# Rodrigops27/MPC-EKF4FastCharge

Hardware: AMD Instinct MI355X
Metric: MPC+EKF control steps/sec (whole batch), Np=5 Nc=2; 1/2/4/8 MI355X (higher is better)
Workload: dtype f64

## Files before the change

### mpc-ekf4fastcharge_amd/csrc/mpcekf_host.cpp

```cpp
#include <hip/hip_runtime.h>

#include <sched.h>

#include <algorithm>
#include <cmath>
#include <condition_variable>
#include <cstdarg>
#include <cstdio>
#include <cstdlib>
#include <cstring>
#include <deque>
#include <mutex>
#include <new>
#include <string>
#include <thread>
#include <vector>

#include "../../include/mpcekf.h"
#include "mpcekf_eig.hpp"
#include "mpcekf_kernels.hpp"
#include "mpcekf_summary.hpp"
#include "mpcekf_thermal.hpp"

using namespace mk;
// ... 142 lines not shown
  int NM = 0, nz = 0, nzp = 0;
  int ncon = 0, ncon_dev = 0, sw = 7;
  bool initialized = false;
  KRom r{};
  KCfg k{};
  KState s{};
  mpcekf_config cfg{};
  double *d_cell_blob = nullptr, *d_plant_blob = nullptr, *d_bulk = nullptr, *d_poly = nullptr;
  double *d_const = nullptr;
  double *d_mb = nullptr;
  bool mb = false;
  double *d_scal = nullptr;
  int *d_int = nullptr;
  double *d_prob = nullptr;
  double *d_zk = nullptr, *d_zbk = nullptr;
  double *d_bnd = nullptr;
  int *d_xm = nullptr;
  double *d_xg = nullptr;
  bool split_cell = false;
  bool quad = false;
  int ekf4_block = 256;
  int *d_ts = nullptr;
  double *d_hist = nullptr;
  long long *d_stamps = nullptr;
  bool wide = false;
  KWide w{};
  double *d_lin = nullptr, *d_zsoc = nullptr;
  std::vector<double> h_lim;
  double *d_lim = nullptr;
  bool percell = false;
  const double *lim() const { return percell ? d_lim : nullptr; }
  double *d_sum = nullptr, *d_sum_reach = nullptr, *d_sum_obs = nullptr;
  char *d_sum_ring = nullptr;
  int32_t sum_slot = -1;
  size_t sum_row() const { return (((size_t)SUM_WIN * (size_t)n * 8) + 255) & ~(size_t)255; }
  double *d_th = nullptr, *d_th_par = nullptr, *d_th_i = nullptr, *d_th_ocv = nullptr;
  int32_t th_nocv = 0;
  double *d_uk1p = nullptr;
  int flush_period = LAZY_H;
  bool flush_roll = false;
  hipStream_t fstream = nullptr;
  hipEvent_t ev_fork = nullptr, ev_join = nullptr;
  bool bounds_side = false;
  hipEvent_t ev_bfork = nullptr, ev_bjoin = nullptr;
  double *d_tmp = nullptr;
  size_t tmp_bytes = 0;
// ... 700 lines not shown
      (rc = dalloc(&X->d_zk, n * (X->nz + 2))) || (rc = dalloc(&X->d_zbk, n * (X->nz + 2))) ||
      (rc = dalloc(&X->d_bnd, n * NBND)) || (rc = dalloc(&X->d_xg, n * 4)) ||
      (rc = hipMalloc((void **)&X->d_xm, n * 4 * sizeof(int)) == hipSuccess ? 0 : MPCEKF_E_HIP) ||
      (rc = dalloc(&X->d_ts, n * NM * 2)) || (rc = dalloc(&X->d_hist, n * LAZY_H * 2)) ||
      (X->mb && (rc = dalloc(&X->d_mb, n * MBREC)))
#ifdef MPCEKF_STAMPS
      || (rc = dalloc(&X->d_stamps, n * NSTAMPS))
#endif
  ) {
    mpcekf_ctx_destroy(X);
    return rc;
  }
  double *sc = X->d_scal;
  s.SOCn = sc; s.SOCp = sc + n; s.x0 = sc + 2 * n; s.S0 = sc + 3 * n; s.priorI = sc + 4 * n;
  s.uk_1 = sc + 5 * n; s.uk = sc + 6 * n; s.vk = sc + 7 * n; s.J_unc = sc + 8 * n; s.J_fin = sc + 9 * n;
  s.warn = X->d_int; s.status = X->d_int + n; s.nviol = X->d_int + 2 * n; s.hflag = X->d_int + 3 * n;
  s.hslow = X->d_int + 4 * n;
  HIPCHK(hipMemset(s.hslow, 0, sizeof(int)));
  s.prob = X->d_prob;
  s.ts_ekf = X->d_ts; s.ts_plant = X->d_ts + n * NM;
  s.hist_p = X->d_hist; s.hist_u = X->d_hist + n * LAZY_H;
  s.mb = X->d_mb;
  s.stamps = X->d_stamps;
  if (X->d_stamps) HIPCHK(hipMemset(X->d_stamps, 0, (size_t)n * NSTAMPS * sizeof(long long)));
  double *cs = X->d_const;
  s.Tc = cs; s.SOC0 = cs + n; s.SOC0n = cs + 2 * n; s.SOC0p = cs + 3 * n;
  if (X->sw != 7 && ((rc = dalloc(&X->d_lin, n * MPCEKF_LIN_SIZE)) || (rc = dalloc(&X->d_zsoc, n)))) {
    mpcekf_ctx_destroy(X);
    return rc;
  }
  if (X->wide) {
    KWide &w = X->w;
    w.Np = cfg->Np; w.Nc = cfg->Nc; w.ncon = X->ncon;
    const size_t nc = (size_t)X->ncon;
    if ((rc = dalloc(&w.prob, n * wide_prob_doubles(w.Np, w.Nc))) || (rc = dalloc(&w.X, nc * n * w.Nc)) ||
        (rc = dalloc(&w.R, (size_t)n * (w.Nc * (w.Nc + 1) / 2))) || (rc = dalloc(&w.K, nc * n)) || (rc = dalloc(&w.hii, nc * n)) || (rc = dalloc(&w.it, n)) ||
        (rc = dalloc(&w.smin, (size_t)w.Nc * w.Nc + 1)) || (rc = dalloc(&X->d_lin, n * MPCEKF_LIN_SIZE)) ||
        (rc = dalloc(&w.q, 1)) || (rc = dalloc(&w.list, n)) || (rc = dalloc(&w.hist, 128)) ||
        (rc = dalloc(&X->d_zsoc, n))) {
      mpcekf_ctx_destroy(X);
      return rc;
    }
    HIPCHK(hipMemset(w.q, 0, sizeof(int)));
    HIPCHK(hipMemset(w.hist, 0, 128 * sizeof(int)));
    HIPCHK(hipMemset(w.it, 0, n * sizeof(int)));
    rc = launch_wide_smin(w, -rom->Ts / (3600 * rom->Q), rom->A, X->stream);
// ... 2 lines not shown
  }
  *out = X;
  return MPCEKF_OK;
}

int mpcekf_ctx_destroy(mpcekf_ctx *X) {
  if (!X) return MPCEKF_OK;
  (void)hipSetDevice(X->device);
  if (X->stream) (void)X->drain();
  if (X->fstream) (void)hipStreamSynchronize(X->fstream);
  delete X->copier;
  X->copier = nullptr;
  for (hipEvent_t e : X->xev) (void)hipEventDestroy(e);
  for (hipEvent_t e : X->ev) (void)hipEventDestroy(e);
  if (X->ev_fork) (void)hipEventDestroy(X->ev_fork);
  if (X->ev_join) (void)hipEventDestroy(X->ev_join);
  if (X->ev_bfork) (void)hipEventDestroy(X->ev_bfork);
  if (X->ev_bjoin) (void)hipEventDestroy(X->ev_bjoin);
  void *ptrs[] = {X->d_prob, X->d_cell_blob, X->d_plant_blob, X->d_bulk, X->d_const, X->d_scal, X->d_int, X->d_zk,
                  X->d_zbk,       X->d_tmp,        X->s.bigx, X->s.ekf,   X->s.lam,   X->d_ts, X->d_hist, X->d_stamps, X->d_bnd, X->d_xm, X->d_xg,
                  X->w.prob, X->w.X, X->w.R, X->w.K, X->w.hii, X->w.it, X->w.smin, X->d_lin, X->d_zsoc, X->d_mb, X->d_uk1p,
                  X->w.q, X->w.list, X->w.hist, X->d_poly, X->d_szk, X->d_sxg, X->d_sxm, X->d_slin, X->d_sv, X->d_zslot,
                  X->d_obs_blob, X->d_obs, X->d_obs_plan, X->d_lim, X->d_sum, X->d_sum_reach, X->d_sum_obs,
                  X->d_sum_ring, X->d_th, X->d_th_par, X->d_th_i, X->d_th_ocv};
  for (void *p : ptrs)
    if (p) (void)hipFree(p);
  for (auto &g : X->graphs) (void)hipGraphExecDestroy(g.exec);
  if (X->h_bounce) (void)hipHostFree(X->h_bounce);
  if (X->fstream) (void)hipStreamDestroy(X->fstream);
  if (X->stream) (void)hipStreamDestroy(X->stream);
  delete X;
  return MPCEKF_OK;
}

int mpcekf_ctx_config(const mpcekf_ctx *X, mpcekf_config *cfg) {
  if (!X || !cfg) return fail(MPCEKF_E_ARG, "ctx_config: null argument");
  *cfg = X->cfg;
  return MPCEKF_OK;
}

int mpcekf_ctx_info(const mpcekf_ctx *X, int64_t *ncells, int32_t *nmodels, int32_t *nz, int32_t *ncon) {
  if (!X) return fail(MPCEKF_E_ARG, "null ctx");
  if (ncells) *ncells = X->n;
  if (nmodels) *nmodels = X->NM;
  if (nz) *nz = X->nz;
  if (ncon) *ncon = X->ncon;
  return MPCEKF_OK;
// ... 26 lines not shown
  if (!X || ((!soc0_pct || !tc_degC) && X->n)) return fail(MPCEKF_E_ARG, "init_cells: null argument");
  HIPCHK(hipSetDevice(X->device));
  const size_t n = (size_t)X->n;
  int rc0 = 0;
  if ((X->n && (rc0 = check_tc(tc_degC, n)))) return rc0;
  std::vector<double> cst(n * 8), sc(n * 10, 0.0);
  for (size_t c = 0; c < n; ++c) {
    double tc = tc_degC[c], soc0 = soc0_pct[c];
    double T = tc + 273.15;
    double z = soc0 / 100;
    cst[0 * n + c] = tc;
    cst[1 * n + c] = z;
    cst[2 * n + c] = host_soc(X, 0, z, T);
    cst[3 * n + c] = host_soc(X, 1, z, T);
    sc[0 * n + c] = cst[2 * n + c];
    sc[1 * n + c] = cst[3 * n + c];
    sc[3 * n + c] = X->cfg.SigmaX0[5];
  }
  HIPCHK(hipMemcpyAsync(X->d_const, cst.data(), cst.size() * 8, hipMemcpyHostToDevice, X->stream));
  HIPCHK(hipMemcpyAsync(X->d_scal, sc.data(), sc.size() * 8, hipMemcpyHostToDevice, X->stream));
  HIPCHK(hipMemsetAsync(X->s.lam, 0, n * X->ncon_dev * 8, X->stream));
  HIPCHK(hipMemsetAsync(X->d_int, 0, n * 4 * sizeof(int), X->stream));
  HIPCHK(hipMemsetAsync(X->d_ts, 0, n * X->NM * 2 * sizeof(int), X->stream));
  int rc = launch_init_state(X->n, X->NM, X->s.ekf, X->s.bigx, X->cfg.SigmaX0, X->stream);
  if (rc) return fail(MPCEKF_E_HIP, "init kernel: %s", hipGetErrorString((hipError_t)rc));
  if (X->mb) {
    std::vector<double> mbs(n * MBREC, 0.0);
    for (size_t c = 0; c < n; ++c)
      for (int p = 0; p <= NX; ++p) mbs[c * MBREC + 6 + p * (NX + 1) + p] = X->cfg.SigmaX0[p];
    HIPCHK(hipMemcpyAsync(X->d_mb, mbs.data(), mbs.size() * 8, hipMemcpyHostToDevice, X->stream));
    HIPCHK(hipStreamSynchronize(X->stream));
  }
  HIPCHK(hipStreamSynchronize(X->stream));
  X->initialized = true;
  return MPCEKF_OK;
}

static int need_init(mpcekf_ctx *X) {
  if (!X) return fail(MPCEKF_E_ARG, "null ctx");
  if (!X->initialized) return fail(MPCEKF_E_STATE, "call mpcekf_init_cells first");
  HIPCHK(hipSetDevice(X->device));
  return MPCEKF_OK;
}

static int lerr(int rc, const char *what) {
  if (rc) return fail(MPCEKF_E_HIP, "%s launch: %s", what, hipGetErrorString((hipError_t)rc));
// ... 274 lines not shown
        q.uk = X->s.uk;
        q.iapp = X->d_th_i;
        q.par = X->d_th_par;
        q.ocv = X->d_th_ocv;
        q.rec = X->d_th;
        q.temp = (double *)row(15, k);
        q.heat = (double *)row(16, k);
        q.n = X->n;
        q.nocv = X->th_nocv;
        q.th0n = X->r.th0n;
        q.th100n = X->r.th100n;
        q.Ts = X->r.Ts;
        if ((rc = lerr(launch_thermal(q, X->stream), "thermal"))) return rc;
      }
    }
    return MPCEKF_OK;
  };
  if (capturing) {
    std::vector<uintptr_t> key = {(uintptr_t)nsteps, (uintptr_t)dtc, (uintptr_t)diag, (uintptr_t)bounds};
    for (const F &e : f) key.push_back((uintptr_t)e.dev);
    key.push_back((uintptr_t)osel.plan);
    key.push_back((uintptr_t)nslots);
    key.push_back((uintptr_t)lim);
    for (int i = 0; i < nslots; ++i) key.push_back((uintptr_t)slots[i]);
    key.push_back((uintptr_t)X->d_th_ocv);
    key.push_back((uintptr_t)X->th_nocv);
    key.push_back((uintptr_t)X->d_th);
    key.push_back((uintptr_t)(sum ? X->d_sum_reach : nullptr));
    key.push_back((uintptr_t)(sum ? X->d_sum : nullptr));
    if ((rc = X->graph_launch(key, run_steps))) return rc;
  } else if ((rc = run_steps())) {
    return rc;
  }
  if (!outputs_on_device)
    for (int i = 0; i < NF; ++i)
      if (f[i].host)
        HIPCHK(hipMemcpyAsync(f[i].host, f[i].dev, per * f[i].width * f[i].esz, hipMemcpyDeviceToHost, X->stream));
  if (nsteps > 0 && f[6].dev)
    HIPCHK(hipMemcpyAsync(X->d_zk, row(6, nsteps - 1), n * nzz * 8, hipMemcpyDeviceToDevice, X->stream));
  if (nsteps > 0 && f[7].dev)
    HIPCHK(hipMemcpyAsync(X->d_zbk, row(7, nsteps - 1), n * nzz * 8, hipMemcpyDeviceToDevice, X->stream));
  HIPCHK(hipStreamSynchronize(X->stream));
  if (X->timing) {
    static const int slot[5] = {MPCEKF_K_PLANT, MPCEKF_K_CELL, MPCEKF_K_BOUNDS, MPCEKF_K_HILD, MPCEKF_K_FLUSH};
    static const int e0[5] = {0, 1, 2, 3, 5};
    for (int k = 0; k < nsteps; ++k)
// ... 992 lines not shown
    HIPCHK(xf.out(scal, dc, n * (size_t)nslots * 8));
  }
  if (warn) HIPCHK(xf.out(warn, X->s.warn, n * 4));
  if (status) HIPCHK(xf.out(status, X->s.status, n * 4));
  return xf.end(async);
}
int mpcekf_get_scalars(mpcekf_ctx *X, const int32_t *slots, int32_t nslots, double *scal, int32_t *warn,
                       int32_t *status) {
  return get_scalars_impl(X, slots, nslots, scal, warn, status, false);
}
int mpcekf_get_scalars_async(mpcekf_ctx *X, const int32_t *slots, int32_t nslots, double *scal, int32_t *warn,
                             int32_t *status) {
  return get_scalars_impl(X, slots, nslots, scal, warn, status, true);
}

int mpcekf_set_state(mpcekf_ctx *X, const mpcekf_state *st) {
  if (X) X->stage_zk = X->stage_lin = X->stage_v = X->stage_obs = false;
  int rc = need_init(X);
  if (rc) return rc;
  if (!st) return fail(MPCEKF_E_ARG, "set_state: null");
  const size_t n = (size_t)X->n, NM = (size_t)X->NM, nc = (size_t)X->ncon, ncd = (size_t)X->ncon_dev;
  if (st->bigX) HIPCHK(hipMemcpyAsync(X->s.bigx, st->bigX, n * NM * 6 * 8, hipMemcpyHostToDevice, X->stream));
  if (st->ekf) HIPCHK(hipMemcpyAsync(X->s.ekf, st->ekf, n * NM * REC * 8, hipMemcpyHostToDevice, X->stream));
  if (st->mb && X->mb) HIPCHK(hipMemcpyAsync(X->d_mb, st->mb, n * MBREC * 8, hipMemcpyHostToDevice, X->stream));
  std::vector<double> sc(st->scal ? n * 8 : 0), lam(st->lambda ? n * ncd : 0);
  std::vector<int> iv(st->warn || st->status ? n * 2 : 0);
  if (!iv.empty() && !(st->warn && st->status)) {
    HIPCHK(hipMemcpyAsync(iv.data(), X->d_int, n * 2 * 4, hipMemcpyDeviceToHost, X->stream));
    HIPCHK(hipStreamSynchronize(X->stream));
  }
  for (size_t c = 0; c < n; ++c) {
    if (st->scal)
      for (int k = 0; k < MPCEKF_NSCAL; ++k) sc[kScalMap[k] * n + c] = st->scal[c * MPCEKF_NSCAL + k];
    if (st->lambda)
      for (size_t i = 0, ci = 0; i < ncd; ++i)
        if (row_enabled(X->cfg.Np, X->cfg.Nc, X->sw, (int)i)) lam[i * n + c] = st->lambda[c * nc + ci++];
    if (st->warn) iv[c] = st->warn[c];
    if (st->status) iv[n + c] = st->status[c];
  }
  if (st->scal) HIPCHK(hipMemcpyAsync(X->d_scal, sc.data(), n * 8 * 8, hipMemcpyHostToDevice, X->stream));
  if (st->lambda) HIPCHK(hipMemcpyAsync(X->s.lam, lam.data(), n * ncd * 8, hipMemcpyHostToDevice, X->stream));
  if (!iv.empty()) HIPCHK(hipMemcpyAsync(X->d_int, iv.data(), n * 2 * 4, hipMemcpyHostToDevice, X->stream));
  HIPCHK(hipStreamSynchronize(X->stream));
  return MPCEKF_OK;
}

// ... 2 lines not shown
```

### mpc-ekf4fastcharge_amd/csrc/mpcekf_kernels.hip

```cpp
#include <hip/hip_runtime.h>

#include <cmath>
#include <cstdlib>
#include <cstdint>
#include <type_traits>

#include "mpcekf_kernels.hpp"
#include "mpcekf_mpc.hpp"
#include "mpcekf_hild.hpp"

#pragma clang fp contract(off)

namespace mk {


#ifdef MPCEKF_STAMPS
#define STAMP(i)                                                                          \
  do {                                                                                    \
    if (io.stamps) io.stamps[(size_t)(i) * s.n + c] = (long long)__builtin_amdgcn_s_memtime(); \
  } while (0)
#define STAMPP(i)                                                                                  \
  do {                                                                                             \
    if (s.stamps) s.stamps[(size_t)(12 + (i)) * s.n + c] = (long long)__builtin_amdgcn_s_memtime(); \
  } while (0)
// ... 273 lines not shown
    two_nearest(Zp, nZ, SOC, a, b);
    iZu = a; iZl = b;
    if (Zp[iZu] < Zp[iZl]) { iZu = b; iZl = a; }
  }
  if (nT > 1) {
    int a, b;
    two_nearest(Tp, nT, Tk, a, b);
    iTu = a; iTl = b;
    if (Tp[iTu] < Tp[iTl]) { iTu = b; iTl = a; }
  }
  double aZ = 0.0, aT = 0.0;
  if (nZ > 1) aZ = (SOC - Zp[iZl]) / (Zp[iZu] - Zp[iZl]);
  if (nT > 1) aT = (Tk - Tp[iTl]) / (Tp[iTu] - Tp[iTl]);
  xi.g[0] = (1 - aT) * (1 - aZ);
  xi.g[1] = (1 - aT) * aZ;
  xi.g[2] = aT * (1 - aZ);
  xi.g[3] = aT * aZ;
  xi.m[0] = iTl * nZ + iZl;
  xi.m[1] = iTl * nZ + iZu;
  xi.m[2] = iTu * nZ + iZl;
  xi.m[3] = iTu * nZ + iZu;
}

__device__ __forceinline__ void load_x(const double *rec, double x[NX]) {
  const double2 *p = reinterpret_cast<const double2 *>(rec);
  double2 a = p[0], b = p[1];
  x[0] = a.x; x[1] = a.y; x[2] = b.x; x[3] = b.y;
  x[4] = rec[4];
}
__device__ __forceinline__ void load_rec(const double *rec, double x[NX], double S[NPK]) {
  const double2 *p = reinterpret_cast<const double2 *>(rec);
  double v[REC];
#pragma unroll
  for (int i = 0; i < REC / 2; ++i) {
    double2 t = p[i];
    v[2 * i] = t.x;
    v[2 * i + 1] = t.y;
  }
#pragma unroll
  for (int i = 0; i < NX; ++i) x[i] = v[i];
#pragma unroll
  for (int i = 0; i < NPK; ++i) S[i] = v[NX + i];
}
__device__ __forceinline__ void store_rec(double *rec, const double x[NX], const double S[NPK]) {
  double2 *p = reinterpret_cast<double2 *>(rec);
  double v[REC];
#pragma unroll
  for (int i = 0; i < NX; ++i) v[i] = x[i];
#pragma unroll
  for (int i = 0; i < NPK; ++i) v[NX + i] = S[i];
#pragma unroll
  for (int i = 0; i < REC / 2; ++i) p[i] = make_double2(v[2 * i], v[2 * i + 1]);
}
__device__ __forceinline__ void load_S(const double *rec, double S[NPK]) {
  S[0] = rec[NX];
  const double2 *p = reinterpret_cast<const double2 *>(rec + NX + 1);
#pragma unroll
  for (int i = 0; i < 7; ++i) {
    double2 t = p[i];
    S[1 + 2 * i] = t.x;
    S[2 + 2 * i] = t.y;
  }
}

__device__ __forceinline__ void jacobi5(double a[NPK], double V[NX * NX]) {
#pragma unroll
  for (int i = 0; i < NX * NX; ++i) V[i] = (i % (NX + 1)) == 0 ? 1.0 : 0.0;
  for (int sweep = 0; sweep < 50; ++sweep) {
    double off = 0.0, dg = 0.0;
#pragma unroll
    for (int p = 0; p < NX; ++p) {
      dg = dg + a[pk(p, p)] * a[pk(p, p)];
#pragma unroll
      for (int q = p + 1; q < NX; ++q) off = off + a[pk(p, q)] * a[pk(p, q)];
    }
    if (!(off > 1e-36 * dg)) break;
#pragma unroll
    for (int p = 0; p < NX - 1; ++p) {
#pragma unroll
      for (int q = p + 1; q < NX; ++q) {
        double apq = a[pk(p, q)];
        if (apq != 0.0) {
          double theta = (a[pk(q, q)] - a[pk(p, p)]) / (2.0 * apq);
          double t;
          if (fabs(theta) > 1e150) {
// ... 994 lines not shown
  const int lo = __builtin_amdgcn_readlane((int)b, l), hi = __builtin_amdgcn_readlane((int)(b >> 32), l);
  return __longlong_as_double(((long long)hi << 32) | (long long)(unsigned)lo);
}
__global__ void __launch_bounds__(256) k_flush(const KRom r, const KCfg cf, const KState s, const int t,
                                               const int new_ts, const int64_t c_lo, const int64_t c_hi) {
  const int NM = r.NM;
  const int lane = threadIdx.x & 63;
  const int64_t nw = (int64_t)gridDim.x * (blockDim.x >> 6);
  const int64_t w0 = ((int64_t)blockIdx.x * blockDim.x + threadIdx.x) >> 6;
  const double W = cf.SigmaW;
  const double *cC = r.bulk_tab, *cP = r.bulk_tab + (size_t)NM * REC;
  for (int m0 = 0; m0 < NM; m0 += 64) {
    const int m = m0 + lane;
    const bool act = m < NM;
    const int mm = act ? m : NM - 1;
    double ce[REC], cp[6];
#pragma unroll
    for (int e = 0; e < REC; ++e) ce[e] = cC[(size_t)mm * REC + e];
#pragma unroll
    for (int e = 0; e < 6; ++e) cp[e] = cP[(size_t)mm * 6 + e];
    struct FCell {
      double hpl, hul, xe[REC], xp[6];
      int tse, tsp;
    };
    auto fload = [&](int64_t c, FCell &F) {
      F.hpl = s.hist_p[(size_t)(lane & (LAZY_H - 1)) * s.n + c];
      F.hul = s.hist_u[(size_t)(lane & (LAZY_H - 1)) * s.n + c];
      F.tse = (act && !(cf.flags & KF_MB)) ? s.ts_ekf[c * NM + m] : t;
      F.tsp = act ? s.ts_plant[c * NM + m] : t;
      const double2 *re = reinterpret_cast<const double2 *>(s.ekf + ((size_t)c * NM + mm) * REC);
      const double2 *rp = reinterpret_cast<const double2 *>(s.bigx + ((size_t)c * NM + mm) * 6);
#pragma unroll
      for (int e = 0; e < REC / 2; ++e) {
        const double2 v = re[e];
        F.xe[2 * e] = v.x;
        F.xe[2 * e + 1] = v.y;
      }
#pragma unroll
      for (int e = 0; e < 3; ++e) {
        const double2 v = rp[e];
        F.xp[2 * e] = v.x;
        F.xp[2 * e + 1] = v.y;
      }
    };
    FCell cur;
    if (c_lo + w0 < c_hi) fload(c_lo + w0, cur);
    for (int64_t c = c_lo + w0; c < c_hi; c += nw) {
      FCell nx;
      if (c + nw < c_hi) fload(c + nw, nx);
      const double hpl = cur.hpl, hul = cur.hul;
      const int tse = cur.tse, tsp = cur.tsp;
      double2 *re = reinterpret_cast<double2 *>(s.ekf + ((size_t)c * NM + mm) * REC);
      double2 *rp = reinterpret_cast<double2 *>(s.bigx + ((size_t)c * NM + mm) * 6);
      double *xe = cur.xe, *xp = cur.xp;
      int kmin = min(tse, tsp);
#pragma unroll
      for (int o = 1; o < 64; o <<= 1) kmin = min(kmin, __shfl_xor(kmin, o));
      for (int k = kmin + 1; k <= t; ++k) {
        const int sl = k & (LAZY_H - 1);
        const double p = rl64(hpl, sl), u = rl64(hul, sl);
        if (k > tse) {
#pragma unroll
          for (int e = 0; e < NX; ++e) xe[e] = __builtin_fma(ce[e], xe[e], p);
#pragma unroll
          for (int e = NX; e < REC; ++e) xe[e] = __builtin_fma(ce[e], xe[e], W);
        }
        if (k > tsp) {
#pragma unroll
          for (int e = 0; e < 6; ++e) xp[e] = __builtin_fma(cp[e], xp[e], u);
        }
      }
      if (tse < t) {
#pragma unroll
        for (int e = 0; e < REC / 2; ++e) re[e] = make_double2(xe[2 * e], xe[2 * e + 1]);
      }
      if (tsp < t) {
#pragma unroll
        for (int e = 0; e < 3; ++e) rp[e] = make_double2(xp[2 * e], xp[2 * e + 1]);
      }
      if (act) {
        s.ts_ekf[c * NM + m] = new_ts;
        s.ts_plant[c * NM + m] = new_ts;
      }
      cur = nx;
    }
  }
}

__device__ __forceinline__ void replay_x(double x[NX], const double *a, int ts, int t, double pt, const KState &s,
                                        int64_t c) {
  if (ts + 1 < t) {
    for (int k0 = ts + 1; k0 < t; k0 += RCH) {
      double p[RCH];
      ring_chunk(s.hist_p, s, c, k0, t - 1, p);
#pragma unroll
      for (int i = 0; i < RCH; ++i)
        if (k0 + i < t)
#pragma unroll
          for (int e = 0; e < NX; ++e) x[e] = __builtin_fma(a[e], x[e], p[i]);
    }
  }
  if (ts < t)
#pragma unroll
    for (int e = 0; e < NX; ++e) x[e] = __builtin_fma(a[e], x[e], pt);
}
__device__ __forceinline__ void replay_S(double S[NPK], const double *a, int ts, int t, double W) {
  for (int k = ts + 1; k <= t; ++k) {
#pragma unroll
    for (int i = 0, pp = 0; pp < NX; ++pp)
#pragma unroll
      for (int q = pp; q < NX; ++q, ++i) S[i] = __builtin_fma(a[NX + i], S[i], W);
  }
}

template <int NZ>
__device__ __forceinline__ void ekf_catch_up4(const KState &s, const CellCtx &cc, int NM, const int m[4], int64_t c,
                                              int t, double W, double pt) {
  int ts[4];
#pragma unroll
  for (int j = 0; j < 4; ++j) ts[j] = s.ts_ekf[c * NM + m[j]];
  bool need[4];
#pragma unroll
  for (int j = 0; j < 4; ++j) {
    need[j] = ts[j] < t;
#pragma unroll
    for (int i = 0; i < j; ++i) need[j] = need[j] && m[i] != m[j];
  }
  if (!(need[0] || need[1] || need[2] || need[3])) return;
  double x[4][NX], S[4][NPK];
#pragma unroll
  for (int j = 0; j < 4; ++j)
    if (need[j]) load_rec(cc.erec + (size_t)m[j] * REC, x[j], S[j]);
#pragma unroll
  for (int j = 0; j < 4; ++j) {
    if (!need[j]) continue;
    const double *a = cc.L + m[j] * cc.stride + NZ * NX + NZ;
    for (int k0 = ts[j] + 1; k0 <= t; k0 += RCH) {
      double p[RCH];
      if (k0 < t) ring_chunk(s.hist_p, s, c, k0, t - 1, p);
#pragma unroll
      for (int i = 0; i < RCH; ++i) {
        const int k = k0 + i;
        if (k > t) break;
// ... 471 lines not shown
    }
    if (io.bnd) io.bnd[BD_M * s.n + c] = -1.0;
    if (io.xm_out) {
#pragma unroll
      for (int j = 0; j < 4; ++j) { io.xm_out[c * 4 + j] = xi.m[j]; io.xg_out[c * 4 + j] = xi.g[j]; }
    }
    } else {
    double x0 = s.x0[c] + s.priorI[c];
    double S0 = s.S0[c] + cf.SigmaW;
    const double SOC0 = s.SOC0[c];
    double SOC = SOC0 - x0 * (r.Ts / (3600 * r.Q));
    STAMP(1);
    get_xind(r.nT, r.nZ, Tp, Zp, cc.T, SOC, xi);
    STAMP(2);
    const int t = io.lazy_t;
    bool dup[4];
    int tsj[4];
    double xr[4][NX], Sr[4][NPK];
#pragma unroll
    for (int j = 0; j < 4; ++j) {
      dup[j] = false;
#pragma unroll
      for (int i = 0; i < j; ++i) dup[j] = dup[j] || xi.m[i] == xi.m[j];
      if (j == 0) load_rec(cc.erec + (size_t)xi.m[j] * REC, xr[j], Sr[j]);
      else load_x(cc.erec + (size_t)xi.m[j] * REC, xr[j]);
      tsj[j] = t ? s.ts_ekf[c * r.NM + xi.m[j]] : 0;
    }
    const double pt = t ? (fplant ? s.priorI[c] : s.hist_p[(size_t)(t % LAZY_H) * s.n + c]) : 0.0;
    run_plant();
    if (planted) vk = vplant;
    if (t) {
#pragma unroll
      for (int j = 0; j < 4; ++j)
        if (!dup[j]) replay_x(xr[j], cc.L + xi.m[j] * cc.stride + NZ * NX + NZ, tsj[j], t, pt, s, c);
#pragma unroll
      for (int j = 1; j < 4; ++j)
#pragma unroll
        for (int i = j - 1; i >= 0; --i)
          if (xi.m[i] == xi.m[j])
#pragma unroll
            for (int k = 0; k < NX; ++k) xr[j][k] = xr[i][k];
    }
    STAMP(3);
    KR kr1;
    vhat = get_vars<NZ>(r, cc, xi, ik, x0, SOC0, warn, st, Z, Zsoc, xr, 0, &kr1);
    STAMP(4);
    if (st & ST_ERROR) {
      s.status[c] = st;
      s.warn[c] = warn;
// ... 18 lines not shown
        row[cI] = acc;
      }
      double acc = 0.0;
#pragma unroll
      for (int cI = 0; cI < NX; ++cI) acc = __builtin_fma(row[cI], ChatV[j][cI], acc);
      St[j] = acc + cf.SigmaV;
#pragma unroll
      for (int k = 0; k < NX; ++k) Lg[j][k] = row[k] / St[j];
    }
    double St0 = C0 * S0 * C0 + cf.SigmaV;
    double L0 = S0 * C0 / St0;
    double res = vk - vhat;
#pragma unroll
    for (int j = 0; j < 4; ++j) {
      launder(St[j]);
#pragma unroll
      for (int k = 0; k < NX; ++k) launder(Lg[j][k]);
    }
    __builtin_amdgcn_sched_barrier(0);
    STAMP(5);
    double xu[4][NX];
    double Sn[NPK];
    auto s_ahead = [&](int j) { return j >= 1 && j < 4 && !dup[j]; };
    if (s_ahead(1)) load_S(cc.erec + (size_t)xi.m[1] * REC, Sn);
#pragma unroll
    for (int j = 0; j < 4; ++j) {
      double *rec = cc.erec + (size_t)xi.m[j] * REC;
      double xj[NX], Sj[NPK];
      if (dup[j]) {
        load_rec(rec, xj, Sj);
      } else {
#pragma unroll
        for (int k = 0; k < NX; ++k) xj[k] = xr[j][k];
        if (j == 0) {
#pragma unroll
          for (int k = 0; k < NPK; ++k) Sj[k] = Sr[j][k];
        } else {
#pragma unroll
          for (int k = 0; k < NPK; ++k) Sj[k] = Sn[k];
        }
        if (t && j > 0) replay_S(Sj, cc.L + xi.m[j] * cc.stride + NZ * NX + NZ, tsj[j], t, cf.SigmaW);
      }
      meas_update_regs<false>(xj, Sj, Lg[j], St[j], res);
      if (j + 1 < 4 && s_ahead(j + 1)) load_S(cc.erec + (size_t)xi.m[j + 1] * REC, Sn);
      store_rec(rec, xj, Sj);
      if (t) s.ts_ekf[c * r.NM + xi.m[j]] = t;
#pragma unroll
      for (int k = 0; k < NX; ++k) xu[j][k] = xj[k];
      __builtin_amdgcn_sched_barrier(0);
    }
    STAMP(6);
    x0 = __builtin_fma(L0, res, x0);
    S0 = S0 - L0 * St0 * L0;
    SOC = SOC0 - x0 * (r.Ts / (3600 * r.Q));
    int m1[4];
#pragma unroll
    for (int j = 0; j < 4; ++j) m1[j] = xi.m[j];
    get_xind(r.nT, r.nZ, Tp, Zp, cc.T, SOC, xi);
    const bool same = m1[0] == xi.m[0] && m1[1] == xi.m[1] && m1[2] == xi.m[2] && m1[3] == xi.m[3] &&
                      !(dup[1] || dup[2] || dup[3]);
    if (!same) {
      if (io.lazy_t) ekf_catch_up4<NZ>(s, cc, r.NM, xi.m, c, io.lazy_t, cf.SigmaW, pt);
#pragma unroll
      for (int j = 0; j < 4; ++j) load_x(cc.erec + (size_t)xi.m[j] * REC, xu[j]);
    }
    STAMP(7);
    vhat = get_vars<NZ>(r, cc, xi, ik, x0, SOC0, warn, st, Z, Zsoc, xu, 0, &kr2);
    have_kr2 = true;
    const int jm = corner_max(xi);
#pragma unroll
    for (int k = 0; k < NX; ++k) xmax[k] = jm == 0 ? xu[0][k] : jm == 1 ? xu[1][k] : jm == 2 ? xu[2][k] : xu[3][k];
    have_xmax = true;
    __builtin_amdgcn_sched_barrier(0);
    STAMP(8);
    s.warn[c] = warn;
    if (st & ST_ERROR) {
      s.status[c] = st;
      s.x0[c] = x0;
      s.S0[c] = S0;
      if (fused) s.uk[c] = NaN;
      fail_outputs();
      return;
    }
    if (io.bnd) {
      double *bd = io.bnd;
      const int64_t n = s.n;
#pragma unroll
// ... 24 lines not shown
    }
    }
  }
  if (!(PARTS & (P_MPC | P_LIN))) return;
  if (!(PARTS & P_EKF) && fused) {
    if (st & ST_ERROR) return;
    vk = s.vk[c];
  }

  Lin L;
  if (io.mode & (MODE_LIN | MODE_FUSED)) {
    double zr[NROLE];
    if (fused && (PARTS & P_EKF)) {
#pragma unroll
      for (int q = 0; q < NROLE; ++q) zr[q] = Z[q];
    } else {
      if (!fused && (st & ST_ERROR)) { fail_outputs(); return; }
#pragma unroll
      for (int q = 0; q < NROLE; ++q) zr[q] = io.zk_in[c * (nz + 2) + r.perm[q]];
      Zsoc = io.zk_in[c * (nz + 2) + nz + 1];
#pragma unroll
      for (int j = 0; j < 4; ++j) { xi.m[j] = io.xm_in[c * 4 + j]; xi.g[j] = io.xg_in[c * 4 + j]; }
    }
    mats_handler<NZ>(r, cc, xi, zr, Zsoc, Tc + 273.15, L, MB ? s.x0[c] : 0.0, xmax, fused && (PARTS & P_EKF) && have_xmax,
                     fused && (PARTS & P_EKF) && have_kr2 ? &kr2 : nullptr);
    if (io.lin_out) lin_store(io.lin_out + c * 35, L);
    if (io.x_out)
#pragma unroll
      for (int q = 0; q < 6; ++q) io.x_out[c * 6 + q] = L.xhat[q];
  }
  STAMP(10);
  if (PARTS & P_LIN) {
    if (fused) {
      double acc = 0.0;
#pragma unroll
      for (int k = 0; k < 6; ++k) acc = acc + L.Cphi[k] * L.xhat[k];
      if (io.phise) io.phise[c] = acc + s.uk[c] * L.Dphi + L.bphi;
      if (io.v) io.v[c] = vk;
      if (io.soc) io.soc[c] = Zsoc;
      if (io.zsoc_out) io.zsoc_out[c] = Zsoc;
    }
    return;
  }

  if (io.mode & (MODE_MPC | MODE_FUSED)) {
    if (!fused) {
      if (st & ST_ERROR) { fail_outputs(); return; }
// ... 309 lines not shown
  return (((0.0 + qbc<0>(v)) + qbc<1>(v)) + qbc<2>(v)) + qbc<3>(v);
}

constexpr int BOUNDS_BLOCK = 1024;
__host__ __device__ inline int bounds_c0_base(const KRom &r) { return r.rom_global ? 0 : r.cell_tab + 1; }
template <int NZ, bool GR>
__global__ void __launch_bounds__(BOUNDS_BLOCK) k_bounds(const KRom r, const KState s, const double *bd, double *zbk) {
  extern __shared__ double lds[];
  if (!GR) stage_lds(lds, r.cell_blob, r.cell_tab);
  __syncthreads();
  const double *L = GR ? r.cell_blob : lds;
  const int64_t gt = (int64_t)blockIdx.x * blockDim.x + threadIdx.x;
  const int64_t n = s.n;
  const int j = (int)(gt & 3);
  const int64_t cq = gt >> 2;
  const int64_t c = cq < n ? cq : n - 1;
  const int nz = r.nz;
  const bool valid = cq < n && bd[BD_M * n + c] >= 0.0;
  const double g = bd[(BD_G + j) * n + c];
  const int m = valid ? (int)bd[(BD_M + j) * n + c] : 0;
  const double *Cm = L + m * r.cell_stride;
  const double S0 = bd[BD_S0 * n + c];
  double S1b[NPK];
  load_S(s.ekf + ((size_t)c * r.NM + (valid ? (int)bd[BD_M * n + c] : 0)) * REC, S1b);
#pragma unroll
  for (int k = 0; k < NX; ++k)
#pragma unroll
    for (int l = k + 1; l < NX; ++l) S1b[pk(k, l)] = 2 * S1b[pk(k, l)];
  ChatK K;
  K.Rfn = bd[(BD_K + 0) * n + c];
  K.Rfp = bd[(BD_K + 1) * n + c];
  K.Rctn = bd[(BD_K + 2) * n + c];
  K.Rctp = bd[(BD_K + 3) * n + c];
  K.dUn0 = bd[(BD_K + 4) * n + c];
  K.dUp3 = bd[(BD_K + 5) * n + c];
  double ChV[NX];
  chat_row(r, K, Cm, g, ChV);
  const double ChV0 = bd[BD_C0 * n + c];
  const double res0n = bd[BD_R0N * n + c], res0p = bd[BD_R0P * n + c];
  const double dUn = bd[BD_DUN * n + c], dUp = bd[BD_DUP * n + c];
  const bool ph0pp = rowf(r, R_PHISE0, G_PPHIS);
  double cph0[NX];
#pragma unroll
  for (int k = 0; k < NX; ++k) {
    double v = g * Cm[R_PHISE0 * NX + k];
    if (ph0pp) v = v + ChV[k];
    cph0[k] = v;
// ... 703 lines not shown
```

### mpc-ekf4fastcharge_amd/csrc/mpcekf_kernels.hpp

```cpp
#pragma once
#include <cstddef>
#include <cstdint>

namespace mk {

constexpr int NX = 5;
constexpr int NPK = 15;
constexpr int NA = 7;
constexpr int REC = 20;
constexpr int MAXT = 8;
constexpr int MAXZ = 40;
constexpr int MAXROWS = 64;
constexpr int NPLANT = 9;
constexpr int PREC = NPLANT * NX + NPLANT + NPLANT + 6;
#ifndef MPCEKF_LAZY_H
#define MPCEKF_LAZY_H 64
#endif
constexpr int LAZY_H = MPCEKF_LAZY_H;
constexpr int MAXTT = 8;
constexpr int MBREC = 42;
constexpr int KF_MB = 1 << 8;

enum { R_IFDL0 = 0, R_IFDL3, R_IF0, R_IF3, R_TH0, R_TH3, R_TE1, R_TEE, R_PHIE, R_PHISE0, R_NPHISE2, NROLE };
enum : unsigned { G_NTH = 1, G_PTH = 2, G_NPHISE = 4, G_PPHISE = 8, G_PHIE = 16, G_PHIE0 = 32, G_THETAE = 64,
// ... 29 lines not shown
  int max_warn, max_hild, flags;
};

enum { LK_REF = 0, LK_U_MAX, LK_U_MIN, LK_DU_MIN, LK_DU_MAX, LK_V_MAX, LK_PHISE_MIN, LK_ZMAX, NLIMK };

struct KState {
  int64_t n;
  double *bigx;
  double *ekf;
  double *SOCn, *SOCp, *x0, *S0, *priorI, *uk_1, *uk, *vk;
  double *lam;
  int *warn, *status;
  double *Tc;
  const double *SOC0, *SOC0n, *SOC0p;
  double *J_unc, *J_fin;
  int *nviol;
  int *hflag;
  int *hslow;
  double *prob;
  double *mb;
  int *ts_ekf, *ts_plant;
  double *hist_p, *hist_u;
  long long *stamps;
};

constexpr int OBS_ROW = 8;
constexpr int OBS_MAXROWS = 32;
enum { OBS_PLAIN = 0, OBS_NTHSS, OBS_PTHSS, OBS_NPHISE, OBS_PPHISE, OBS_PHIE, OBS_THETAE, OBS_PPHIS };
enum { OBS_S_NEGSOC = 0, OBS_S_POSSOC, OBS_S_CELLSOC };
struct KObs {
  const double *blob;
  int stride, tab, tablen, len;
  int global;
  int nobs, slot_phie0;
  unsigned desc[OBS_MAXROWS];
  double *rec;
};

enum { OBS_SRC_NEGSOC = -1, OBS_SRC_POSSOC = -2, OBS_SRC_CELLSOC = -3, OBS_SRC_PHIE0 = -4, OBS_SRC_VCELL = -5 };
enum { OBS_NEED_V = 1,
       OBS_NEED_UN = 2,
       OBS_NEED_UP = 4 };
struct KObsSel {
  const int *plan;
  int nsel, need;
  double *out;
};
// ... 98 lines not shown
```

Measured before the change: 252.0 million.

## Cache four active EKF corner records in a coalesced hot buffer

Adds a per-cell hot buffer holding the four currently active interpolation-corner EKF records in a struct-of-arrays layout (stride n), plus their model indices and timestamps. The cell kernel reads and writes these hot slots when the corner set is unchanged, and writes them back to the main per-model record array when the corners change. The lazy flush, xmax lookup and bounds kernels are updated to consult the hot slots. The aim is coalesced global memory access instead of scattered record loads, at the cost of extra index checks, write-back traffic on corner changes, and more complexity around state consistency.

```diff
diff --git a/mpc-ekf4fastcharge_amd/csrc/mpcekf_host.cpp b/mpc-ekf4fastcharge_amd/csrc/mpcekf_host.cpp
--- a/mpc-ekf4fastcharge_amd/csrc/mpcekf_host.cpp
+++ b/mpc-ekf4fastcharge_amd/csrc/mpcekf_host.cpp
@@ -188,6 +188,12 @@
   int ekf4_block = 256;
   int *d_ts = nullptr;
   double *d_hist = nullptr;
+  double *d_hot = nullptr;
+  int *d_hot_i = nullptr;
+  int hot_clear() {
+    if (d_hot_i) HIPCHK(hipMemsetAsync(d_hot_i, 0xFF, (size_t)n * 4 * sizeof(int), stream));
+    return MPCEKF_OK;
+  }
   long long *d_stamps = nullptr;
   bool wide = false;
   KWide w{};
@@ -934,6 +940,25 @@
   s.hist_p = X->d_hist; s.hist_u = X->d_hist + n * LAZY_H;
   s.mb = X->d_mb;
   s.stamps = X->d_stamps;
+  {
+    bool hot = true;
+    if (const char *e = std::getenv("MPCEKF_HOT_CORNERS")) hot = std::atoi(e) != 0;
+    if (hot && !X->mb && !X->quad && !X->flush_roll && n > 0) {
+      if (hipMalloc((void **)&X->d_hot, n * 4 * REC * sizeof(double)) != hipSuccess ||
+          hipMalloc((void **)&X->d_hot_i, n * 8 * sizeof(int)) != hipSuccess) {
+        (void)hipGetLastError();
+        if (X->d_hot) (void)hipFree(X->d_hot);
+        if (X->d_hot_i) (void)hipFree(X->d_hot_i);
+        X->d_hot = nullptr;
+        X->d_hot_i = nullptr;
+      } else {
+        s.hot_rec = X->d_hot;
+        s.hot_m = X->d_hot_i;
+        s.hot_ts = X->d_hot_i + n * 4;
+        if ((rc = X->hot_clear())) { mpcekf_ctx_destroy(X); return rc; }
+      }
+    }
+  }
   if (X->d_stamps) HIPCHK(hipMemset(X->d_stamps, 0, (size_t)n * NSTAMPS * sizeof(long long)));
   double *cs = X->d_const;
   s.Tc = cs; s.SOC0 = cs + n; s.SOC0n = cs + 2 * n; s.SOC0p = cs + 3 * n;
@@ -982,7 +1007,7 @@
                   X->w.prob, X->w.X, X->w.R, X->w.K, X->w.hii, X->w.it, X->w.smin, X->d_lin, X->d_zsoc, X->d_mb, X->d_uk1p,
                   X->w.q, X->w.list, X->w.hist, X->d_poly, X->d_szk, X->d_sxg, X->d_sxm, X->d_slin, X->d_sv, X->d_zslot,
                   X->d_obs_blob, X->d_obs, X->d_obs_plan, X->d_lim, X->d_sum, X->d_sum_reach, X->d_sum_obs,
-                  X->d_sum_ring, X->d_th, X->d_th_par, X->d_th_i, X->d_th_ocv};
+                  X->d_sum_ring, X->d_th, X->d_th_par, X->d_th_i, X->d_th_ocv, X->d_hot, X->d_hot_i};
   for (void *p : ptrs)
     if (p) (void)hipFree(p);
   for (auto &g : X->graphs) (void)hipGraphExecDestroy(g.exec);
@@ -1055,6 +1080,7 @@
   HIPCHK(hipMemsetAsync(X->s.lam, 0, n * X->ncon_dev * 8, X->stream));
   HIPCHK(hipMemsetAsync(X->d_int, 0, n * 4 * sizeof(int), X->stream));
   HIPCHK(hipMemsetAsync(X->d_ts, 0, n * X->NM * 2 * sizeof(int), X->stream));
+  if ((rc0 = X->hot_clear())) return rc0;
   int rc = launch_init_state(X->n, X->NM, X->s.ekf, X->s.bigx, X->cfg.SigmaX0, X->stream);
   if (rc) return fail(MPCEKF_E_HIP, "init kernel: %s", hipGetErrorString((hipError_t)rc));
   if (X->mb) {
@@ -1375,6 +1401,7 @@
     key.push_back((uintptr_t)osel.plan);
     key.push_back((uintptr_t)nslots);
     key.push_back((uintptr_t)lim);
+    key.push_back((uintptr_t)X->s.hot_rec);
     for (int i = 0; i < nslots; ++i) key.push_back((uintptr_t)slots[i]);
     key.push_back((uintptr_t)X->d_th_ocv);
     key.push_back((uintptr_t)X->th_nocv);
@@ -2413,6 +2440,7 @@
   const size_t n = (size_t)X->n, NM = (size_t)X->NM, nc = (size_t)X->ncon, ncd = (size_t)X->ncon_dev;
   if (st->bigX) HIPCHK(hipMemcpyAsync(X->s.bigx, st->bigX, n * NM * 6 * 8, hipMemcpyHostToDevice, X->stream));
   if (st->ekf) HIPCHK(hipMemcpyAsync(X->s.ekf, st->ekf, n * NM * REC * 8, hipMemcpyHostToDevice, X->stream));
+  if ((rc = X->hot_clear())) return rc;
   if (st->mb && X->mb) HIPCHK(hipMemcpyAsync(X->d_mb, st->mb, n * MBREC * 8, hipMemcpyHostToDevice, X->stream));
   std::vector<double> sc(st->scal ? n * 8 : 0), lam(st->lambda ? n * ncd : 0);
   std::vector<int> iv(st->warn || st->status ? n * 2 : 0);
diff --git a/mpc-ekf4fastcharge_amd/csrc/mpcekf_kernels.hip b/mpc-ekf4fastcharge_amd/csrc/mpcekf_kernels.hip
--- a/mpc-ekf4fastcharge_amd/csrc/mpcekf_kernels.hip
+++ b/mpc-ekf4fastcharge_amd/csrc/mpcekf_kernels.hip
@@ -319,18 +319,18 @@
   xi.m[3] = iTu * nZ + iZu;
 }
 
-__device__ __forceinline__ void load_x(const double *rec, double x[NX]) {
+__device__ __forceinline__ void load_x(const double *rec, double x[NX], size_t st = 1) {
   const double2 *p = reinterpret_cast<const double2 *>(rec);
-  double2 a = p[0], b = p[1];
+  double2 a = p[0], b = p[st];
   x[0] = a.x; x[1] = a.y; x[2] = b.x; x[3] = b.y;
-  x[4] = rec[4];
-}
-__device__ __forceinline__ void load_rec(const double *rec, double x[NX], double S[NPK]) {
+  x[4] = reinterpret_cast<const double *>(p + 2 * st)[0];
+}
+__device__ __forceinline__ void load_rec(const double *rec, double x[NX], double S[NPK], size_t st = 1) {
   const double2 *p = reinterpret_cast<const double2 *>(rec);
   double v[REC];
 #pragma unroll
   for (int i = 0; i < REC / 2; ++i) {
-    double2 t = p[i];
+    double2 t = p[i * st];
     v[2 * i] = t.x;
     v[2 * i + 1] = t.y;
   }
@@ -339,7 +339,7 @@
 #pragma unroll
   for (int i = 0; i < NPK; ++i) S[i] = v[NX + i];
 }
-__device__ __forceinline__ void store_rec(double *rec, const double x[NX], const double S[NPK]) {
+__device__ __forceinline__ void store_rec(double *rec, const double x[NX], const double S[NPK], size_t st = 1) {
   double2 *p = reinterpret_cast<double2 *>(rec);
   double v[REC];
 #pragma unroll
@@ -347,17 +347,20 @@
 #pragma unroll
   for (int i = 0; i < NPK; ++i) v[NX + i] = S[i];
 #pragma unroll
-  for (int i = 0; i < REC / 2; ++i) p[i] = make_double2(v[2 * i], v[2 * i + 1]);
-}
-__device__ __forceinline__ void load_S(const double *rec, double S[NPK]) {
-  S[0] = rec[NX];
-  const double2 *p = reinterpret_cast<const double2 *>(rec + NX + 1);
+  for (int i = 0; i < REC / 2; ++i) p[i * st] = make_double2(v[2 * i], v[2 * i + 1]);
+}
+__device__ __forceinline__ void load_S(const double *rec, double S[NPK], size_t st = 1) {
+  const double2 *p = reinterpret_cast<const double2 *>(rec);
+  S[0] = reinterpret_cast<const double *>(p + 2 * st)[1];
 #pragma unroll
   for (int i = 0; i < 7; ++i) {
-    double2 t = p[i];
+    double2 t = p[(3 + i) * st];
     S[1 + 2 * i] = t.x;
     S[2 + 2 * i] = t.y;
   }
+}
+__device__ __forceinline__ double *hot_slot(const KState &s, int j, int64_t c) {
+  return s.hot_rec + 2 * ((size_t)j * HOT_PAIRS * (size_t)s.n + (size_t)c);
 }
 
 __device__ __forceinline__ void jacobi5(double a[NPK], double V[NX * NX]) {
@@ -1398,17 +1401,27 @@
     struct FCell {
       double hpl, hul, xe[REC], xp[6];
       int tse, tsp;
+      int slot;
     };
     auto fload = [&](int64_t c, FCell &F) {
       F.hpl = s.hist_p[(size_t)(lane & (LAZY_H - 1)) * s.n + c];
       F.hul = s.hist_u[(size_t)(lane & (LAZY_H - 1)) * s.n + c];
-      F.tse = (act && !(cf.flags & KF_MB)) ? s.ts_ekf[c * NM + m] : t;
+      F.slot = -1;
+      if (s.hot_m) {
+#pragma unroll
+        for (int j = 0; j < 4; ++j)
+          if (act && s.hot_m[(size_t)j * s.n + c] == m) F.slot = j;
+      }
+      const int *tp = F.slot >= 0 ? s.hot_ts + (size_t)F.slot * s.n + c : s.ts_ekf + c * NM + mm;
+      F.tse = (act && !(cf.flags & KF_MB)) ? *tp : t;
       F.tsp = act ? s.ts_plant[c * NM + m] : t;
-      const double2 *re = reinterpret_cast<const double2 *>(s.ekf + ((size_t)c * NM + mm) * REC);
+      const double2 *re = reinterpret_cast<const double2 *>(F.slot >= 0 ? hot_slot(s, F.slot, c)
+                                                                        : s.ekf + ((size_t)c * NM + mm) * REC);
+      const size_t rst = F.slot >= 0 ? (size_t)s.n : 1;
       const double2 *rp = reinterpret_cast<const double2 *>(s.bigx + ((size_t)c * NM + mm) * 6);
 #pragma unroll
       for (int e = 0; e < REC / 2; ++e) {
-        const double2 v = re[e];
+        const double2 v = re[e * rst];
         F.xe[2 * e] = v.x;
         F.xe[2 * e + 1] = v.y;
       }
@@ -1446,10 +1459,11 @@
           for (int e = 0; e < 6; ++e) xp[e] = __builtin_fma(cp[e], xp[e], u);
         }
       }
-      if (tse < t) {
+      if (tse < t || cur.slot >= 0) {
 #pragma unroll
         for (int e = 0; e < REC / 2; ++e) re[e] = make_double2(xe[2 * e], xe[2 * e + 1]);
       }
+      if (cur.slot >= 0) s.hot_m[(size_t)cur.slot * s.n + c] = -1;
       if (tsp < t) {
 #pragma unroll
         for (int e = 0; e < 3; ++e) rp[e] = make_double2(xp[2 * e], xp[2 * e + 1]);
@@ -1491,10 +1505,10 @@
 
 template <int NZ>
 __device__ __forceinline__ void ekf_catch_up4(const KState &s, const CellCtx &cc, int NM, const int m[4], int64_t c,
-                                              int t, double W, double pt) {
+                                              int t, double W, double pt, const bool held[4]) {
   int ts[4];
 #pragma unroll
-  for (int j = 0; j < 4; ++j) ts[j] = s.ts_ekf[c * NM + m[j]];
+  for (int j = 0; j < 4; ++j) ts[j] = held[j] ? t : s.ts_ekf[c * NM + m[j]];
   bool need[4];
 #pragma unroll
   for (int j = 0; j < 4; ++j) {
@@ -2012,9 +2026,38 @@
       dup[j] = false;
 #pragma unroll
       for (int i = 0; i < j; ++i) dup[j] = dup[j] || xi.m[i] == xi.m[j];
-      if (j == 0) load_rec(cc.erec + (size_t)xi.m[j] * REC, xr[j], Sr[j]);
-      else load_x(cc.erec + (size_t)xi.m[j] * REC, xr[j]);
-      tsj[j] = t ? s.ts_ekf[c * r.NM + xi.m[j]] : 0;
+    }
+    const size_t hn = (size_t)s.n;
+    const bool win = s.hot_m != nullptr && t != 0;
+    bool hot = false, hit = false;
+    if (win) {
+      int hm[4];
+#pragma unroll
+      for (int j = 0; j < 4; ++j) hm[j] = s.hot_m[j * hn + c];
+      hot = !(dup[1] || dup[2] || dup[3]);
+      hit = hot && hm[0] == xi.m[0] && hm[1] == xi.m[1] && hm[2] == xi.m[2] && hm[3] == xi.m[3];
+      if (!hit) {
+#pragma unroll 1
+        for (int j = 0; j < 4; ++j) {
+          const int mh = s.hot_m[j * hn + c];
+          if (mh < 0) continue;
+          double xh[NX], Sh[NPK];
+          load_rec(hot_slot(s, j, c), xh, Sh, hn);
+          store_rec(cc.erec + (size_t)mh * REC, xh, Sh);
+          s.ts_ekf[c * r.NM + mh] = s.hot_ts[j * hn + c];
+          if (!hot) s.hot_m[j * hn + c] = -1;
+        }
+      }
+    }
+    const size_t rst = hit ? hn : 1;
+    const size_t wst = hot ? hn : 1;
+    auto rrec = [&](int j) -> const double * { return hit ? hot_slot(s, j, c) : cc.erec + (size_t)xi.m[j] * REC; };
+#pragma unroll
+    for (int j = 0; j < 4; ++j) {
+      if (j == 0) load_rec(rrec(j), xr[j], Sr[j], rst);
+      else load_x(rrec(j), xr[j], rst);
+      const int *tp = hit ? s.hot_ts + j * hn + c : s.ts_ekf + c * r.NM + xi.m[j];
+      tsj[j] = t ? *tp : 0;
     }
     const double pt = t ? (fplant ? s.priorI[c] : s.hist_p[(size_t)(t % LAZY_H) * s.n + c]) : 0.0;
     run_plant();
@@ -2079,7 +2122,7 @@
     double xu[4][NX];
     double Sn[NPK];
     auto s_ahead = [&](int j) { return j >= 1 && j < 4 && !dup[j]; };
-    if (s_ahead(1)) load_S(cc.erec + (size_t)xi.m[1] * REC, Sn);
+    if (s_ahead(1)) load_S(rrec(1), Sn, rst);
 #pragma unroll
     for (int j = 0; j < 4; ++j) {
       double *rec = cc.erec + (size_t)xi.m[j] * REC;
@@ -2099,9 +2142,12 @@
         if (t && j > 0) replay_S(Sj, cc.L + xi.m[j] * cc.stride + NZ * NX + NZ, tsj[j], t, cf.SigmaW);
       }
       meas_update_regs<false>(xj, Sj, Lg[j], St[j], res);
-      if (j + 1 < 4 && s_ahead(j + 1)) load_S(cc.erec + (size_t)xi.m[j + 1] * REC, Sn);
-      store_rec(rec, xj, Sj);
-      if (t) s.ts_ekf[c * r.NM + xi.m[j]] = t;
+      if (j + 1 < 4 && s_ahead(j + 1)) load_S(rrec(j + 1), Sn, rst);
+      store_rec(hot ? hot_slot(s, j, c) : rec, xj, Sj, wst);
+      if (t) {
+        *(hot ? s.hot_ts + j * hn + c : s.ts_ekf + c * r.NM + xi.m[j]) = t;
+        if (hot && !hit) s.hot_m[j * hn + c] = xi.m[j];
+      }
 #pragma unroll
       for (int k = 0; k < NX; ++k) xu[j][k] = xj[k];
       __builtin_amdgcn_sched_barrier(0);
@@ -2117,9 +2163,26 @@
     const bool same = m1[0] == xi.m[0] && m1[1] == xi.m[1] && m1[2] == xi.m[2] && m1[3] == xi.m[3] &&
                       !(dup[1] || dup[2] || dup[3]);
     if (!same) {
-      if (io.lazy_t) ekf_catch_up4<NZ>(s, cc, r.NM, xi.m, c, io.lazy_t, cf.SigmaW, pt);
-#pragma unroll
-      for (int j = 0; j < 4; ++j) load_x(cc.erec + (size_t)xi.m[j] * REC, xu[j]);
+      bool held[4];
+      double xn[4][NX];
+#pragma unroll
+      for (int j = 0; j < 4; ++j) {
+        held[j] = false;
+#pragma unroll
+        for (int i = 0; i < 4; ++i)
+          if (hot && m1[i] == xi.m[j]) {
+            held[j] = true;
+#pragma unroll
+            for (int k = 0; k < NX; ++k) xn[j][k] = xu[i][k];
+          }
+      }
+      if (io.lazy_t) ekf_catch_up4<NZ>(s, cc, r.NM, xi.m, c, io.lazy_t, cf.SigmaW, pt, held);
+#pragma unroll
+      for (int j = 0; j < 4; ++j) {
+        if (!held[j]) load_x(cc.erec + (size_t)xi.m[j] * REC, xn[j]);
+#pragma unroll
+        for (int k = 0; k < NX; ++k) xu[j][k] = xn[j][k];
+      }
     }
     STAMP(7);
     vhat = get_vars<NZ>(r, cc, xi, ik, x0, SOC0, warn, st, Z, Zsoc, xu, 0, &kr2);
@@ -2190,7 +2253,19 @@
 #pragma unroll
       for (int j = 0; j < 4; ++j) { xi.m[j] = io.xm_in[c * 4 + j]; xi.g[j] = io.xg_in[c * 4 + j]; }
     }
-    mats_handler<NZ>(r, cc, xi, zr, Zsoc, Tc + 273.15, L, MB ? s.x0[c] : 0.0, xmax, fused && (PARTS & P_EKF) && have_xmax,
+    if constexpr (!(PARTS & P_EKF) && !MB) {
+      if (fused && s.hot_m && io.lazy_t) {
+        int mx;
+        (void)corner_max(xi, &mx);
+#pragma unroll
+        for (int j = 0; j < 4; ++j)
+          if (!have_xmax && s.hot_m[(size_t)j * s.n + c] == mx) {
+            load_x(hot_slot(s, j, c), xmax, (size_t)s.n);
+            have_xmax = true;
+          }
+      }
+    }
+    mats_handler<NZ>(r, cc, xi, zr, Zsoc, Tc + 273.15, L, MB ? s.x0[c] : 0.0, xmax, fused && have_xmax,
                      fused && (PARTS & P_EKF) && have_kr2 ? &kr2 : nullptr);
     if (io.lin_out) lin_store(io.lin_out + c * 35, L);
     if (io.x_out)
@@ -2546,7 +2621,14 @@
   const double *Cm = L + m * r.cell_stride;
   const double S0 = bd[BD_S0 * n + c];
   double S1b[NPK];
-  load_S(s.ekf + ((size_t)c * r.NM + (valid ? (int)bd[BD_M * n + c] : 0)) * REC, S1b);
+  const int m0 = valid ? (int)bd[BD_M * n + c] : 0;
+  int hslot = -1;
+  if (s.hot_m) {
+#pragma unroll
+    for (int i = 0; i < 4; ++i)
+      if (valid && s.hot_m[(size_t)i * n + c] == m0) hslot = i;
+  }
+  load_S(hslot >= 0 ? hot_slot(s, hslot, c) : s.ekf + ((size_t)c * r.NM + m0) * REC, S1b, hslot >= 0 ? (size_t)n : 1);
 #pragma unroll
   for (int k = 0; k < NX; ++k)
 #pragma unroll
diff --git a/mpc-ekf4fastcharge_amd/csrc/mpcekf_kernels.hpp b/mpc-ekf4fastcharge_amd/csrc/mpcekf_kernels.hpp
--- a/mpc-ekf4fastcharge_amd/csrc/mpcekf_kernels.hpp
+++ b/mpc-ekf4fastcharge_amd/csrc/mpcekf_kernels.hpp
@@ -75,7 +75,10 @@
   int *ts_ekf, *ts_plant;
   double *hist_p, *hist_u;
   long long *stamps;
-};
+  double *hot_rec;
+  int *hot_m, *hot_ts;
+};
+constexpr int HOT_PAIRS = REC / 2;
 
 constexpr int OBS_ROW = 8;
 constexpr int OBS_MAXROWS = 32;
```

New measurement: 267.2 million, median of 6. 1.06x the previous value.
